# mumianyuxin/M3DSSD

Measured on AMD Instinct MI355X. Metric: images/sec at 1280x384 bs=8, 1/2/4/8 MI355X; 3D-box Linf vs ref, higher is better.
Workload: dtype f32; 1 GPU; BASELINE.json configs[1]: full M3d_inference_align (DLA-34 + DCNv2 align + ANAB) forward + decode + top-3000 + NMS, bs=8/GPU, 1280x384, fp32, random-init synthetic weights and frames; per_gpu_batch=8, global_batch=8, parallelism=dp1 (batch sharded, 1 all-gather of [B,40,14] detections)

## Files before the change

### include/m3dssd_hip.h

```cpp
#ifndef M3DSSD_HIP_H
#define M3DSSD_HIP_H

#include <stdint.h>

#ifdef __cplusplus
extern "C" {
#endif

typedef void *m3d_stream_t;

enum {
    M3D_OK = 0,
    M3D_E_ARG = -1,
    M3D_E_HIP = -2,
    M3D_E_WORKSPACE = -3
};

const char *m3d_last_error(void);
#define M3D_ABI_VERSION 5
int m3d_abi_version(void);
const char *m3d_source_hashes(void);

typedef struct m3d_conv_desc {
    const float *in;
// ... 9 lines not shown
    int out_nchw;
    long long out_img_stride;
    const float *scale;
    const float *shift;
    const float *res;
    int res_cs;
    int res_mode;
    int act;
    int sigmoid_from;
    const float *dcn_offmask;
    int dcn_om_cs;
    float *splitk_ws;
    long long splitk_ws_bytes;
} m3d_conv_desc;

int m3d_conv2d_forward(const m3d_conv_desc *d, m3d_stream_t stream);
int m3d_conv2d_splitk_plan(const m3d_conv_desc *d, int *splits, long long *ws_bytes);

int m3d_conv_wave_applicable(const m3d_conv_desc *d);
int m3d_conv_wave_splitk_plan(const m3d_conv_desc *d, int *splits, long long *ws_bytes);
int m3d_conv_wave_forward(const m3d_conv_desc *d, m3d_stream_t stream);
int m3d_conv_wave_forward_wgsplit(const m3d_conv_desc *d, m3d_stream_t stream);
int m3d_conv_wave_wgsplit_width(const m3d_conv_desc *d, int *slices, int *width);

int m3d_wino_conv3x3_forward(const m3d_conv_desc *d, m3d_stream_t stream);
int m3d_wino_conv3x3_variant(const m3d_conv_desc *d);
int m3d_wino_conv3x3_splitk_plan(const m3d_conv_desc *d, int *splits, long long *ws_bytes);
int m3d_wino_conv3x3_forward_ex(const m3d_conv_desc *d, int variant, m3d_stream_t stream);
int m3d_wino44_applicable(const m3d_conv_desc *d);
int m3d_wino44_conv3x3_forward(const m3d_conv_desc *d, m3d_stream_t stream);
int m3d_wino44_conv3x3_forward_ex(const m3d_conv_desc *d, int nb, m3d_stream_t stream);
int m3d_wino44_kpair(const m3d_conv_desc *d);
int m3d_wino44_splitk_plan(const m3d_conv_desc *d, int *splits, long long *ws_bytes);
int m3d_wino44_conv3x3_forward_touch(const m3d_conv_desc *d, int nb, const void *touch, long long touch_bytes, m3d_stream_t stream);

int m3d_cache_touch(const void *p, long long bytes, m3d_stream_t stream);
int m3d_upload_indirect(const void *const *src_slot, void *dst, long long bytes, m3d_stream_t stream);

int m3d_conv2d_tile(const m3d_conv_desc *d, int *bm, int *bn, int *bk, int *grid);

typedef struct m3d_conv_bf16_desc {
    const void *in;
    int in_cs;
    int N, H, W, Cin;
    const void *wgt;
    long long wgt_img_stride;
// ... 355 lines not shown
```

### m3dssd_amd/_hip.py

```python
import ctypes
import os
import subprocess

_HERE = os.path.dirname(os.path.abspath(__file__))
CSRC = os.path.join(_HERE, "csrc")
SO_PATH = os.environ.get("M3D_HIP_LIB") or os.path.join(CSRC, "build", "libm3dssd_hip.so")
HEADER = os.path.join(os.path.dirname(_HERE), "include", "m3dssd_hip.h")

c_int, c_float, c_ll, c_void_p = ctypes.c_int, ctypes.c_float, ctypes.c_longlong, ctypes.c_void_p


class ConvDesc(ctypes.Structure):
    _fields_ = [
        ("inp", c_void_p), ("in_cs", c_int),
        ("N", c_int), ("H", c_int), ("W", c_int), ("Cin", c_int),
        ("wgt", c_void_p), ("wgt_img_stride", c_ll),
        ("Cout", c_int), ("Cout_pad", c_int),
        ("kh", c_int), ("kw", c_int), ("stride", c_int), ("pad", c_int), ("dil", c_int),
        ("Ho", c_int), ("Wo", c_int),
        ("out", c_void_p), ("out_cs", c_int), ("out_nchw", c_int), ("out_img_stride", c_ll),
        ("scale", c_void_p), ("shift", c_void_p),
        ("res", c_void_p), ("res_cs", c_int), ("res_mode", c_int),
        ("act", c_int), ("sigmoid_from", c_int),
        ("dcn_offmask", c_void_p), ("dcn_om_cs", c_int),
# ... 109 lines not shown
    "m3d_upsample2x_add_bf16": (c_int, [P, c_int, P, P, c_int, P, c_int] + [c_int] * 4 + [P]),
    "m3d_f32_to_bf16": (c_int, [P, P, c_ll, P]),
    "m3d_softmax_rows_bf16": (c_int, [P, c_int, c_int, c_int, P, c_int, P]),
    "m3d_head_mlp_forward": (c_int, [ctypes.POINTER(MlpDesc), P]),
    "m3d_head_mlp_forward_batched": (c_int, [ctypes.POINTER(MlpDesc), c_int, P]),
    "m3d_head_mlp_forward_rows": (c_int, [ctypes.POINTER(MlpDesc), c_int, P, P, ctypes.c_uint, P]),
    "m3d_wino_conv3x3_forward": (c_int, [ctypes.POINTER(ConvDesc), P]),
    "m3d_wino_conv3x3_forward_ex": (c_int, [ctypes.POINTER(ConvDesc), c_int, P]),
    "m3d_wino_conv3x3_splitk_plan": (c_int, [ctypes.POINTER(ConvDesc), ctypes.POINTER(c_int), ctypes.POINTER(c_ll)]),
    "m3d_wino_conv3x3_variant": (c_int, [ctypes.POINTER(ConvDesc)]),
    "m3d_wino44_applicable": (c_int, [ctypes.POINTER(ConvDesc)]),
    "m3d_wino44_conv3x3_forward": (c_int, [ctypes.POINTER(ConvDesc), P]),
    "m3d_wino44_conv3x3_forward_ex": (c_int, [ctypes.POINTER(ConvDesc), c_int, P]),
    "m3d_wino44_kpair": (c_int, [ctypes.POINTER(ConvDesc)]),
    "m3d_wino44_conv3x3_forward_touch": (c_int, [ctypes.POINTER(ConvDesc), c_int, P, c_ll, P]),
    "m3d_cache_touch": (c_int, [P, c_ll, P]),
    "m3d_upload_indirect": (c_int, [P, P, c_ll, P]),
    "m3d_wino44_splitk_plan": (c_int, [ctypes.POINTER(ConvDesc), ctypes.POINTER(c_int), ctypes.POINTER(c_ll)]),
    "m3d_conv_wave_applicable": (c_int, [ctypes.POINTER(ConvDesc)]),
    "m3d_conv_wave_splitk_plan": (c_int, [ctypes.POINTER(ConvDesc), ctypes.POINTER(c_int), ctypes.POINTER(c_ll)]),
    "m3d_conv_wave_forward": (c_int, [ctypes.POINTER(ConvDesc), P]),
    "m3d_conv_wave_forward_wgsplit": (c_int, [ctypes.POINTER(ConvDesc), P]),
    "m3d_conv_wave_wgsplit_width": (c_int, [ctypes.POINTER(ConvDesc), ctypes.POINTER(c_int), ctypes.POINTER(c_int)]),
    "m3d_conv2d_tile": (c_int, [ctypes.POINTER(ConvDesc)] + [ctypes.POINTER(c_int)] * 4),
    "m3d_conv2d_splitk_plan": (c_int, [ctypes.POINTER(ConvDesc), ctypes.POINTER(c_int), ctypes.POINTER(c_ll)]),
    "m3d_dcn_v2_workspace_bytes": (c_ll, [c_int] * 10),
    "m3d_dcn_v2_workspace_bytes_grouped": (c_ll, [c_int] * 11),
    "m3d_dcn_v2_forward": (c_int, [P] * 6 + [c_int] * 14 + [P, c_ll, P]),
    "m3d_dcn_v2_backward_workspace_bytes": (c_ll, [c_int] * 11),
    "m3d_dcn_v2_backward": (c_int, [P] * 10 + [c_int] * 14 + [P, c_ll, P]),
    "m3d_dcn_v2_workspace_bytes_bf16": (c_ll, [c_int] * 11),
    "m3d_dcn_v2_forward_bf16": (c_int, [P, P, P, P, c_int, P, c_int, P] + [c_int] * 14 + [P, c_ll, P]),
    "m3d_dcn_v2_backward_workspace_bytes_bf16": (c_ll, [c_int] * 11),
    "m3d_dcn_v2_backward_bf16": (c_int, [P, P, P, c_int, P, c_int, P] + [P] * 5 + [c_int] * 14 + [P, c_ll, P]),
    "m3d_dcn_v2_psroi_pooling_workspace_bytes": (c_ll, [c_int] * 10),
    "m3d_dcn_v2_psroi_pooling_forward": (c_int, [P] * 5 + [c_int] * 8 + [c_float] + [c_int] * 5 + [c_float, P, c_ll, P]),
    "m3d_dcn_v2_psroi_pooling_backward": (c_int, [P] * 6 + [c_int] * 8 + [c_float] + [c_int] * 5 + [c_float, P, c_ll, P]),
    "m3d_rpn_loss_workspace_bytes": (c_ll, [c_int, c_ll]),
    "m3d_rpn_targets": (c_int, [P, c_int, c_int, c_int, P, c_int, P, c_int, c_int, P, P, c_int, P, P, P, P, P, c_ll, P]),
    "m3d_rpn_loss": (c_int, [P, c_int, c_int, c_int, P, c_int, P, c_int, c_int, P, P, P, c_int, P, P, P, P, P, P, P, P, P, P, c_ll, P]),
    "m3d_pack_conv_weight": (c_int, [P, P] + [c_int] * 6 + [P]),
    "m3d_nchw_to_nhwc": (c_int, [P, P] + [c_int] * 5 + [P]),
    "m3d_nhwc_to_nchw": (c_int, [P, c_int, P] + [c_int] * 4 + [P]),
    "m3d_stem_conv7x7": (c_int, [P, P, P, P, P] + [c_int] * 4 + [P]),
    "m3d_refine_3d": (c_int, [P, P, c_int, c_int, P, P, ctypes.c_double, c_int, ctypes.c_double, ctypes.c_double, P, P]),
    "m3d_refine_3d_ex": (c_int, [P, P, c_int, c_int, P, P, P, P, ctypes.c_double, c_int, ctypes.c_double, ctypes.c_double, P, P]),
# ... 96 lines not shown
```

### m3dssd_amd/csrc/dcn_wave.hip

```cpp

#include <type_traits>

#include "common.h"

struct ConvWaveArgs {
    const float *in, *wfrag, *scale, *shift, *res, *om;
    float *out;
    int in_cs, out_cs, res_cs, om_cs;
    int H, W, Cin, Ho, Wo, HoWo, Cout;
    int kh, kw, stride, pad, dil;
    int M, KG, tiles_n;
    int act, res_mode, sigmoid_from;
    int vec_out;
    long long w_img_stride;
    unsigned in_bytes, out_bytes, res_bytes, w_bytes;
    float *ws;
    int splits, ss_per, base_waves;
    unsigned ws_bytes;
#ifdef CONV_TRACE
    long long *trace;
#endif
};


#ifdef CONV_TRACE
static long long *g_conv_trace = nullptr;
extern "C" void m3d_conv_wave_set_trace(void *buf) { g_conv_trace = (long long *)buf; }
static int g_conv_variant = 0;
extern "C" void m3d_conv_wave_set_variant(int v) { g_conv_variant = v; }
#define TRACE_INIT() long long *trp = (a.trace && threadIdx.x < 64) ? a.trace + (size_t)blockIdx.x * 128 : nullptr; int tri = 0
#define TRACE() do { if (trp && lane == 0 && tri < 128) trp[tri++] = __builtin_readcyclecounter(); } while (0)
#else
#define TRACE_INIT()
#define TRACE()
#endif

template <bool DEFORM, int NT, int NCQ = 4, int WPE = (DEFORM ? 2 : 3), int S = 1>
__global__ __launch_bounds__(64 * S) __attribute__((amdgpu_waves_per_eu(WPE))) void conv_wave_kernel(const ConvWaveArgs a)
{
    __shared__ __attribute__((aligned(16))) float tileS[S * 32 * 32];
    __shared__ __attribute__((aligned(16))) float tapst[(DEFORM ? 9 : 1) * 32 * 8];
    const int lane = threadIdx.x & 63, l31 = lane & 31, h = lane >> 5;
    const int wv = S > 1 ? __builtin_amdgcn_readfirstlane((int)threadIdx.x >> 6) : 0;
    float *const tileA = tileS + wv * 1024;
    const int gp = lane >> 3, gc = lane & 7;
    TRACE_INIT();
    TRACE();
    int blk;
    {
        const int nblk = gridDim.x, bid = blockIdx.x;
        const int q = nblk >> 3, r = nblk & 7, xcd = bid & 7, loc = bid >> 3;
        blk = (xcd < r ? xcd * (q + 1) : r * (q + 1) + (xcd - r) * q) + loc;
    }
    int split = wv;
    if (S == 1 && a.splits > 1) {
        split = blk / a.base_waves;
        blk -= split * a.base_waves;
    }
    const int bm = blk / a.tiles_n, bn = blk - bm * a.tiles_n;
    const int m0 = bm * 32;
    const int KK = a.kh * a.kw, C32 = a.Cin / 32;
    const bool idle = S > 1 && wv >= a.splits;
// ... 255 lines not shown
                    const float *p = &tileS[px[q] * 32 + 4 * c4];
                    f32x4 v = *reinterpret_cast<const f32x4 *>(p);
#pragma unroll
                    for (int s = 1; s < S; ++s)
                        if (s < a.splits) v = v + *reinterpret_cast<const f32x4 *>(p + s * 1024);
                    v = conv_epi_affine(v, scv[nt], shv[nt], a.res ? rv[q] : v, a.res != nullptr, a.res_mode);
                    v = conv_epi_act4(v, c, a.sigmoid_from, tile_sig, slope);
                    if (full) {
                        __builtin_amdgcn_raw_buffer_store_b128(__builtin_bit_cast(u32x4, v), rout, oq[q] + (unsigned)c * 4u, 0, 0);
                    } else {
#pragma unroll
                        for (int e = 0; e < 4; ++e) {
                            const float pe = v[e];
                            __builtin_amdgcn_raw_buffer_store_b32(__builtin_bit_cast(unsigned, pe), rout,
                                                                  c + e < a.Cout ? oq[q] + (unsigned)(c + e) * 4u : M3D_BUF_OOB, 0, 0);
                        }
                    }
                }
            }
        }
        TRACE();
        return;
    }
    if (a.splits > 1) {
        const __amdgpu_buffer_rsrc_t rws = make_rsrc(a.ws, a.ws_bytes);
        const unsigned sbase = (unsigned)split * (unsigned)a.M;
        const unsigned cpad = (unsigned)(a.tiles_n * 32 * NT);
#pragma unroll
        for (int nt = 0; nt < NT; ++nt) {
            const unsigned co = (unsigned)(n0 + nt * 32 + l31);
#pragma unroll
            for (int r = 0; r < 16; ++r) {
                const int m = mb + (r & 3) + 8 * (r >> 2);
                const unsigned oo = m < a.M ? ((sbase + (unsigned)m) * cpad + co) * 4u : M3D_BUF_OOB;
                const float pv = acc[nt][r];
                __builtin_amdgcn_raw_buffer_store_b32(__builtin_bit_cast(unsigned, pv), rws, oo, 0, 0);
            }
        }
        return;
    }
    if (a.vec_out) {
        const float slope = a.act == 1 ? M3D_LEAKY_SLOPE : 1.f;
        const int pr = lane >> 3, c4 = lane & 7;
        unsigned oq[4], rq[4];
#pragma unroll
        for (int q = 0; q < 4; ++q) {
            const int m = m0 + pr + 8 * q;
            oq[q] = m < a.M ? (unsigned)m * (unsigned)a.out_cs * 4u : M3D_BUF_OOB;
            rq[q] = m < a.M ? (unsigned)m * (unsigned)a.res_cs * 4u : M3D_BUF_OOB;
        }
        f32x4 scv[NT], shv[NT];
#pragma unroll
        for (int nt = 0; nt < NT; ++nt) {
            const int c = n0 + nt * 32 + 4 * c4;
            scv[nt] = f32x4{1.f, 1.f, 1.f, 1.f};
            shv[nt] = f32x4{0.f, 0.f, 0.f, 0.f};
            if (c + 3 < a.Cout) {
                if (a.scale) scv[nt] = *reinterpret_cast<const f32x4 *>(a.scale + c);
                if (a.shift) shv[nt] = *reinterpret_cast<const f32x4 *>(a.shift + c);
            } else {
#pragma unroll
                for (int e = 0; e < 4; ++e)
                    if (c + e < a.Cout) {
                        if (a.scale) scv[nt][e] = a.scale[c + e];
                        if (a.shift) shv[nt][e] = a.shift[c + e];
                    }
            }
        }
#pragma unroll
        for (int nt = 0; nt < NT; ++nt) {
            const int c = n0 + nt * 32 + 4 * c4;
            f32x4 rv[4];
            if (a.res) {
#pragma unroll
                for (int q = 0; q < 4; ++q) {
                    if (c + 3 < a.Cout) {
                        rv[q] = __builtin_bit_cast(f32x4, __builtin_amdgcn_raw_buffer_load_b128(rres, rq[q] + (unsigned)c * 4u, 0, 0));
                    } else {
#pragma unroll
                        for (int e = 0; e < 4; ++e)
                            rv[q][e] = __builtin_bit_cast(float, __builtin_amdgcn_raw_buffer_load_b32(
                                rres, c + e < a.Cout ? rq[q] + (unsigned)(c + e) * 4u : M3D_BUF_OOB, 0, 0));
                    }
                }
            }
#pragma unroll
            for (int r = 0; r < 16; ++r) tileA[((r & 3) + 8 * (r >> 2) + 4 * h) * 32 + l31] = acc[nt][r];
            const bool tile_sig = a.sigmoid_from >= 0 && n0 + nt * 32 + 31 >= a.sigmoid_from;
#pragma unroll
            for (int q = 0; q < 4; ++q) {
                f32x4 v = *reinterpret_cast<const f32x4 *>(&tileA[(pr + 8 * q) * 32 + 4 * c4]);
                v = conv_epi_affine(v, scv[nt], shv[nt], a.res ? rv[q] : v, a.res != nullptr, a.res_mode);
                v = conv_epi_act4(v, c, a.sigmoid_from, tile_sig, slope);
                if (c + 3 < a.Cout) {
                    __builtin_amdgcn_raw_buffer_store_b128(__builtin_bit_cast(u32x4, v), rout, oq[q] + (unsigned)c * 4u, 0, 0);
                } else {
#pragma unroll
                    for (int e = 0; e < 4; ++e) {
                        const float pe = v[e];
                        __builtin_amdgcn_raw_buffer_store_b32(__builtin_bit_cast(unsigned, pe), rout,
                                                              c + e < a.Cout ? oq[q] + (unsigned)(c + e) * 4u : M3D_BUF_OOB, 0, 0);
                    }
                }
            }
        }
        TRACE();
        return;
    }
#pragma unroll
    for (int nt = 0; nt < NT; ++nt) {
        const int co = n0 + nt * 32 + l31;
        const bool cok = co < a.Cout;
        const float sc = (cok && a.scale) ? a.scale[co] : 1.f;
        const float sh = (cok && a.shift) ? a.shift[co] : 0.f;
        float rv[16];
        if (a.res) {
#pragma unroll
            for (int r = 0; r < 16; ++r) {
                const int m = mb + (r & 3) + 8 * (r >> 2);
                const unsigned ro = (cok && m < a.M) ? ((unsigned)m * (unsigned)a.res_cs + (unsigned)co) * 4u : M3D_BUF_OOB;
                rv[r] = __builtin_bit_cast(float, __builtin_amdgcn_raw_buffer_load_b32(rres, ro, 0, 0));
            }
        }
#pragma unroll
        for (int r = 0; r < 16; ++r) {
            const int m = mb + (r & 3) + 8 * (r >> 2);
            float v = conv_epi_affine(acc[nt][r], sc, sh, a.res ? rv[r] : 0.f, a.res != nullptr, a.res_mode);
            v = conv_epi_act(v, a.sigmoid_from >= 0 && co >= a.sigmoid_from, a.act == 1 ? M3D_LEAKY_SLOPE : 1.f);
            const unsigned oo = (cok && m < a.M) ? ((unsigned)m * (unsigned)a.out_cs + (unsigned)co) * 4u : M3D_BUF_OOB;
            __builtin_amdgcn_raw_buffer_store_b32(__builtin_bit_cast(unsigned, v), rout, oo, 0, 0);
        }
    }
    TRACE();
}

static int conv_wave_plan(const m3d_conv_desc *d, bool enforce_min, int *splits, int *ss_per, bool allow32 = false)
{
    *splits = 1;
    *ss_per = d->kh * d->kw * (d->Cin / 32);
    if (d->out_nchw) return 0;
    if (d->dcn_offmask && d->kh * d->kw > 9) return 0;
    if (d->Cin % 32 != 0 || d->Cout_pad % 32 != 0) return 0;
    if (d->Cout_pad % 64 != 0 && (!allow32 || d->dcn_offmask || d->wgt_img_stride)) return 0;
    const int cw = d->Cout_pad % 128 == 0 ? 128 : (d->Cout_pad % 64 == 0 ? 64 : 32);
    if (d->wgt_img_stride && (d->Ho * d->Wo) % 32 != 0) return 0;
    const long long M = (long long)d->N * d->Ho * d->Wo;
    const long long base = ((M + 31) / 32) * (d->Cout_pad / cw);
    if (base >= (1ll << 28)) return 0;
    static const int wave_min = m3d_env_int("M3D_CONV_WAVE_MIN", 900);
    static const int dcn_min = m3d_env_int("M3D_DCN_WAVE_MIN", 1500);
    static const int splitk = m3d_env_int("M3D_CONV_WAVE_SPLITK", 1);
    const long long need = d->dcn_offmask ? dcn_min : wave_min;
    const int nss = *ss_per;
    if (base < need && splitk && d->splitk_ws) {
        int s = (int)((1800 + base - 1) / base);
        if (s > nss / 4) s = nss / 4;
// ... 6 lines not shown
    if (enforce_min && base * *splits < need) { *splits = 1; *ss_per = nss; return 0; }
    return (int)(base * *splits);
}

extern "C" int m3d_conv_wave_applicable(const m3d_conv_desc *d)
{
    int s, p;
    return d ? conv_wave_plan(d, true, &s, &p) : 0;
}

extern "C" int m3d_conv_wave_splitk_plan(const m3d_conv_desc *d, int *splits, long long *ws_bytes)
{
    M3D_REQUIRE(d && splits && ws_bytes, "conv_wave_splitk_plan: null pointer");
    m3d_conv_desc t = *d;
    static float dummy;
    t.splitk_ws = &dummy;
    int p;
    const int waves = conv_wave_plan(&t, true, splits, &p, true);
    if (waves == 0) *splits = 1;
    *ws_bytes = (*splits > 1 && d->Cout_pad % 64 == 0) ? (long long)*splits * d->N * d->Ho * d->Wo * d->Cout_pad * 4 : 0;
    return M3D_OK;
}

template <bool DEFORM, int NT>
static void launch_wgsplit(const ConvWaveArgs &a, int S, int wgs, hipStream_t stream)
{
    constexpr int WPE = DEFORM ? 2 : 3;
    switch (S) {
    case 2: hipLaunchKernelGGL((conv_wave_kernel<DEFORM, NT, 4, WPE, 2>), dim3(wgs), dim3(128), 0, stream, a); break;
    case 4: hipLaunchKernelGGL((conv_wave_kernel<DEFORM, NT, 4, WPE, 4>), dim3(wgs), dim3(256), 0, stream, a); break;
    default: hipLaunchKernelGGL((conv_wave_kernel<DEFORM, NT, 4, WPE, 8>), dim3(wgs), dim3(512), 0, stream, a); break;
    }
}

static int conv_wave_run(const m3d_conv_desc *d_, hipStream_t stream, bool wgsplit)
{
    M3D_REQUIRE(d_ && d_->in && d_->wgt && d_->out, "conv_wave: null pointer");
    m3d_conv_desc dd = *d_;
    static float dummy;
    if (wgsplit) { dd.splitk_ws = &dummy; dd.splitk_ws_bytes = 0; }
    const m3d_conv_desc *d = &dd;
    int splits = 1, ss_per = 0;
    const int waves = conv_wave_plan(d, false, &splits, &ss_per, wgsplit);
    M3D_REQUIRE(waves > 0, "conv_wave: needs Cin %% 32 == 0, Cout_pad %% 64 == 0 (%% 32: plain, shared weights, wgsplit entry), NHWC output, "
                           "Ho*Wo %% 32 == 0 with per-image weights");
    const int ho = (d->H + 2 * d->pad - (d->dil * (d->kh - 1) + 1)) / d->stride + 1;
    const int wo = (d->W + 2 * d->pad - (d->dil * (d->kw - 1) + 1)) / d->stride + 1;
    M3D_REQUIRE(ho == d->Ho && wo == d->Wo, "conv_wave: Ho/Wo mismatch");
    M3D_REQUIRE(d->in_cs % 32 == 0 && d->in_cs >= d->Cin && ((uintptr_t)d->in & 127) == 0 && ((uintptr_t)d->wgt & 15) == 0,
                "conv_wave: the input view must be 128-byte aligned with in_cs %% 32 == 0");
    const long long M = (long long)d->N * d->Ho * d->Wo;
    M3D_REQUIRE(!d->wgt_img_stride || (d->wgt_img_stride % 4 == 0 && d->stride == 1 && d->Ho == d->H && d->Wo == d->W),
                "conv_wave: per-image weights need an image-aligned 16-byte stride and a same-size output");
    M3D_REQUIRE((long long)d->N * d->H * d->W * d->in_cs * 4 < (1ll << 31) && M * d->out_cs * 4 < (1ll << 31) &&
                M * d->res_cs * 4 < (1ll << 31) && (long long)d->Cout_pad * d->kh * d->kw * d->Cin * 4 < (1ll << 31),
                "conv_wave: views must be < 2 GiB");
    ConvWaveArgs a;
    a.in = d->in; a.wfrag = d->wgt; a.scale = d->scale; a.shift = d->shift; a.res = d->res; a.om = d->dcn_offmask;
    a.out = d->out;
    a.in_cs = d->in_cs; a.out_cs = d->out_cs; a.res_cs = d->res_cs; a.om_cs = d->dcn_om_cs;
    a.H = d->H; a.W = d->W; a.Cin = d->Cin; a.Ho = d->Ho; a.Wo = d->Wo; a.HoWo = d->Ho * d->Wo; a.Cout = d->Cout;
    a.kh = d->kh; a.kw = d->kw; a.stride = d->stride; a.pad = d->pad; a.dil = d->dil;
    const int cw = d->Cout_pad % 128 == 0 ? 128 : (d->Cout_pad % 64 == 0 ? 64 : 32);
    a.M = (int)M; a.KG = d->kh * d->kw * d->Cin / 8; a.tiles_n = d->Cout_pad / cw;
    a.act = d->act; a.res_mode = d->res_mode; a.sigmoid_from = d->sigmoid_from; a.w_img_stride = d->wgt_img_stride;
    static const int vec_epi = m3d_env_int("M3D_WAVE_VEC_EPILOGUE", 1);
    a.vec_out = vec_epi && d->out_cs % 4 == 0 && ((uintptr_t)d->out & 15) == 0 &&
                (!d->res || (d->res_cs % 4 == 0 && ((uintptr_t)d->res & 15) == 0)) &&
                (!d->scale || ((uintptr_t)d->scale & 15) == 0) && (!d->shift || ((uintptr_t)d->shift & 15) == 0);
    a.in_bytes = (unsigned)((long long)d->N * d->H * d->W * d->in_cs * 4);
    a.out_bytes = (unsigned)(M * d->out_cs * 4);
    a.res_bytes = (unsigned)(M * d->res_cs * 4);
    a.w_bytes = (unsigned)((long long)cw * d->kh * d->kw * d->Cin * 4);
#ifdef CONV_TRACE
    a.trace = g_conv_trace;
#endif
    a.ws = nullptr; a.splits = 1; a.ss_per = ss_per; a.base_waves = waves; a.ws_bytes = 0;
    if (splits > 1 && wgsplit) {
        const int S = splits <= 2 ? 2 : (splits <= 4 ? 4 : 8);
        M3D_REQUIRE(splits <= 8, "conv_wave: %d K slices do not fit a workgroup", splits);
        a.splits = splits; a.base_waves = waves / splits;
        if (cw == 128) {
            if (d->dcn_offmask) launch_wgsplit<true, 4>(a, S, a.base_waves, stream);
            else launch_wgsplit<false, 4>(a, S, a.base_waves, stream);
        } else if (cw == 64) {
            if (d->dcn_offmask) launch_wgsplit<true, 2>(a, S, a.base_waves, stream);
            else launch_wgsplit<false, 2>(a, S, a.base_waves, stream);
        } else {
            launch_wgsplit<false, 1>(a, S, a.base_waves, stream);
        }
        M3D_LAUNCH_CHECK();
        return M3D_OK;
    }
    if (splits > 1) {
        const long long need = (long long)splits * M * d->Cout_pad * 4;
        M3D_REQUIRE(need <= d->splitk_ws_bytes && need < (1ll << 31) && ((uintptr_t)d->splitk_ws & 15) == 0,
                    "conv_wave: split-K workspace too small (%lld bytes, see m3d_conv_wave_splitk_plan), >= 2 GiB or misaligned",
                    d->splitk_ws_bytes);
        a.ws = d->splitk_ws; a.splits = splits; a.base_waves = waves / splits; a.ws_bytes = (unsigned)need;
    }
// ... 32 lines not shown

extern "C" int m3d_conv_wave_forward(const m3d_conv_desc *d, m3d_stream_t stream)
{
    return conv_wave_run(d, (hipStream_t)stream, false);
}

extern "C" int m3d_conv_wave_wgsplit_width(const m3d_conv_desc *d, int *slices, int *width)
{
    M3D_REQUIRE(d && slices && width, "conv_wave_wgsplit_width: null pointer");
    m3d_conv_desc t = *d;
    static float dummy;
    t.splitk_ws = &dummy;
    int p;
    const int waves = conv_wave_plan(&t, false, slices, &p, true);
    M3D_REQUIRE(waves > 0 && *slices <= 8, "conv_wave_wgsplit_width: the wave kernel does not apply to this descriptor");
    *width = *slices <= 1 ? 1 : (*slices <= 2 ? 2 : (*slices <= 4 ? 4 : 8));
    return M3D_OK;
}

extern "C" int m3d_conv_wave_forward_wgsplit(const m3d_conv_desc *d, m3d_stream_t stream)
{
    return conv_wave_run(d, (hipStream_t)stream, true);
}
```

### m3dssd_amd/engine.py

```python
import ctypes
import math
import os

import numpy as np
import torch

from . import _hip
from ._hip import ConvDesc, MlpDesc
from .config import model_flags

BN_EPS = 1e-5
SELECT_KEYS = os.environ.get("M3D_SELECT_KEYS", "1") != "0"
SPARSE_HEADS_MAX_FRACTION = 0.5
PSP_SIZES = (1, 4, 8, 16)
BACKBONE_CHANNELS = {"dla34": (16, 32, 64, 128, 256, 512), "dla102": (16, 32, 128, 256, 512, 1024)}
DLA102_LEVELS = (1, 1, 1, 3, 4, 1)


def _rup(a, b):
    return (a + b - 1) // b * b


class View:
    __slots__ = ("t", "ptr", "n", "h", "w", "c", "cs", "keep")
# ... 482 lines not shown
        l0 = self._buf(plan, B, H, W, 16, name="level0")
        if P.get("level0.wino44") is not None and H % 4 == 0 and W % 4 == 0 and os.environ.get("M3D_LEVEL0_WINO44", "1") != "0":
            pc0 = P["level0"]
            self._op(plan, "level0", "wino44_c16", lambda st: _hip.check(L.m3d_conv3x3_c16_wino(
                s0.ptr, s0.cs, P["level0.wino44"].data_ptr(), pc0.scale.data_ptr(), pc0.shift.data_ptr(), l0.ptr, l0.cs,
                B, H, W, st)), flops=2.0 * B * H * W * 16 * 144, nbytes=B * H * W * 32 * 4)
        elif P["level0.direct"] is not None and os.environ.get("M3D_LEVEL0_IGEMM", "0") != "1":
            pc0 = P["level0"]
            self._op(plan, "level0", "conv3x3_c16", lambda st: _hip.check(L.m3d_conv3x3_c16(
                s0.ptr, s0.cs, P["level0.direct"].data_ptr(), pc0.scale.data_ptr(), pc0.shift.data_ptr(), l0.ptr, l0.cs,
                B, H, W, st)), flops=2.0 * B * H * W * 16 * 144, nbytes=B * H * W * 32 * 4)
        else:
            self._conv(plan, "level0", P["level0"], s0, l0, 1, 1, act=1)
        l1 = self._buf(plan, B, H // 2, W // 2, 32, name="level1")
        self._conv(plan, "level1", P["level1"], l0, l1, 2, 1, act=1)

        def maxpool(name, x, out):
            self._op(plan, name, "maxpool", lambda st: _hip.check(L.m3d_maxpool2x2(
                x.ptr, x.cs, out.ptr, out.cs, x.n, x.h, x.w, x.c, st)), nbytes=x.n * x.h * x.w * x.c * 5)

        if self.back_bone == "dla102":
            l3, l4, l5 = self._dla102_levels(plan, l1, maxpool)
        else:
            def block(p, x, res, out, stride):
                co = P[p + ".conv1"].cout
                t = self._buf(plan, B, out.h, out.w, co)
                self._conv(plan, p + ".conv1", P[p + ".conv1"], x, t, stride, 1, act=1)
                self._conv(plan, p + ".conv2", P[p + ".conv2"], t, out, 1, 1, act=1, res=res)

            def tree1(p, x, co, stride, out, bottom=None):
                h, w = x.h // stride, x.w // stride
                cat = self._buf(plan, B, h, w, 2 * co)
                x2v, x1v = cat.slice(0, co), cat.slice(co, co)
                if stride == 1:
                    bottom = x
                elif bottom is None:
                    bottom = self._buf(plan, B, h, w, x.c)
                    maxpool(p + ".downsample", x, bottom)
                if (p + ".project") in P:
                    res = self._buf(plan, B, h, w, co)
                    self._conv(plan, p + ".project", P[p + ".project"], bottom, res, 1, 0, act=0)
                else:
                    res = bottom
                block(p + ".tree1", x, res, x1v, stride)
                block(p + ".tree2", x1v, x1v, x2v, 1)
                self._conv(plan, p + ".root", P[p + ".root"], cat, out, 1, 0, act=1)

            l2 = self._buf(plan, B, H // 4, W // 4, 64, name="level2")
            tree1(b + ".level2", l1, 64, 2, l2)

            def tree2(p, x, co, out):
                ci = x.c
                h, w = x.h // 2, x.w // 2
                catb = self._buf(plan, B, h, w, 2 * co + ci + co)
                bottom = catb.slice(2 * co, ci)
                X1 = catb.slice(2 * co + ci, co)
                maxpool(p + ".downsample", x, bottom)
                tree1(p + ".tree1", x, co, 2, X1, bottom=bottom)
                x2v, x1v = catb.slice(0, co), catb.slice(co, co)
                block(p + ".tree2.tree1", X1, X1, x1v, 1)
                block(p + ".tree2.tree2", x1v, x1v, x2v, 1)
                self._conv(plan, p + ".tree2.root", P[p + ".tree2.root"], catb, out, 1, 0, act=1)

            l3 = self._buf(plan, B, H // 8, W // 8, 128, name="level3")
            tree2(b + ".level3", l2, 128, l3)
            l4 = self._buf(plan, B, H // 16, W // 16, 256, name="level4")
            tree2(b + ".level4", l3, 256, l4)
            l5 = self._buf(plan, B, H // 32, W // 32, 512, name="level5")
            h5, w5 = H // 32, W // 32
            cat5 = self._buf(plan, B, h5, w5, 1024 + 256)
            bottom5 = cat5.slice(1024, 256)
            maxpool(b + ".level5.downsample", l4, bottom5)
            res5 = self._buf(plan, B, h5, w5, 512)
            self._conv(plan, b + ".level5.project", P[b + ".level5.project"], bottom5, res5, 1, 0, act=0)
            block(b + ".level5.tree1", l4, res5, cat5.slice(512, 512), 2)
            block(b + ".level5.tree2", cat5.slice(512, 512), cat5.slice(512, 512), cat5.slice(0, 512), 1)
            self._conv(plan, b + ".level5.root", P[b + ".level5.root"], cat5, l5, 1, 0, act=1)

        def deform(p, x, out):
            om = self._buf(plan, B, x.h, x.w, 27, 28)
            self._conv(plan, p + ".offset_mask", P[p + ".om"], x, om, 1, 1, act=0, sigmoid_from=18)
# ... 493 lines not shown
```

Measured before the change: 1556 images/sec.

## Fuse DLA tree entry maxpool, 1x1 projection and stride-2 conv1 into one kernel

Adds an ENTRY variant of the wave conv kernel that runs the stride-2 3x3 conv1 and then, in a second pass, builds the 2x2 max-pooled input from the conv1 gather taps. It feeds that pooled tile straight into the 1x1 projection MFMA and optionally writes the pooled map when a later concat needs it. This replaces three launches (maxpool, project, conv1) with one and avoids writing and re-reading the pooled map when it is only used internally. The cost is a longer and more complex kernel with higher register pressure, and it only applies to unsplit plans with even H and W; otherwise the three-launch path is kept.

```diff
diff --git a/include/m3dssd_hip.h b/include/m3dssd_hip.h
--- a/include/m3dssd_hip.h
+++ b/include/m3dssd_hip.h
@@ -55,6 +55,8 @@
 int m3d_conv_wave_forward(const m3d_conv_desc *d, m3d_stream_t stream);
 int m3d_conv_wave_forward_wgsplit(const m3d_conv_desc *d, m3d_stream_t stream);
 int m3d_conv_wave_wgsplit_width(const m3d_conv_desc *d, int *slices, int *width);
+int m3d_conv_wave_tree_entry_forward(const m3d_conv_desc *conv1, const m3d_conv_desc *project, float *bottom, int bottom_cs,
+                                     m3d_stream_t stream);
 
 int m3d_wino_conv3x3_forward(const m3d_conv_desc *d, m3d_stream_t stream);
 int m3d_wino_conv3x3_variant(const m3d_conv_desc *d);
diff --git a/m3dssd_amd/_hip.py b/m3dssd_amd/_hip.py
--- a/m3dssd_amd/_hip.py
+++ b/m3dssd_amd/_hip.py
@@ -155,6 +155,7 @@
     "m3d_conv_wave_forward": (c_int, [ctypes.POINTER(ConvDesc), P]),
     "m3d_conv_wave_forward_wgsplit": (c_int, [ctypes.POINTER(ConvDesc), P]),
     "m3d_conv_wave_wgsplit_width": (c_int, [ctypes.POINTER(ConvDesc), ctypes.POINTER(c_int), ctypes.POINTER(c_int)]),
+    "m3d_conv_wave_tree_entry_forward": (c_int, [ctypes.POINTER(ConvDesc), ctypes.POINTER(ConvDesc), P, c_int, P]),
     "m3d_conv2d_tile": (c_int, [ctypes.POINTER(ConvDesc)] + [ctypes.POINTER(c_int)] * 4),
     "m3d_conv2d_splitk_plan": (c_int, [ctypes.POINTER(ConvDesc), ctypes.POINTER(c_int), ctypes.POINTER(c_ll)]),
     "m3d_dcn_v2_workspace_bytes": (c_ll, [c_int] * 10),
diff --git a/m3dssd_amd/csrc/dcn_wave.hip b/m3dssd_amd/csrc/dcn_wave.hip
--- a/m3dssd_amd/csrc/dcn_wave.hip
+++ b/m3dssd_amd/csrc/dcn_wave.hip
@@ -22,6 +22,18 @@
 #endif
 };
 
+struct ConvEntryArgs : ConvWaveArgs {
+    const float *p_wfrag, *p_scale, *p_shift;
+    float *p_out, *bottom;
+    int p_out_cs, bottom_cs, p_KG, p_vec_out;
+    unsigned p_out_bytes, bottom_bytes, p_w_bytes;
+};
+
+struct ConvWaveEpi {
+    const float *scale, *shift, *res;
+    int out_cs, res_cs, act, res_mode, sigmoid_from, vec_out;
+};
+
 
 #ifdef CONV_TRACE
 static long long *g_conv_trace = nullptr;
@@ -35,9 +47,12 @@
 #define TRACE()
 #endif
 
-template <bool DEFORM, int NT, int NCQ = 4, int WPE = (DEFORM ? 2 : 3), int S = 1>
-__global__ __launch_bounds__(64 * S) __attribute__((amdgpu_waves_per_eu(WPE))) void conv_wave_kernel(const ConvWaveArgs a)
-{
+template <bool DEFORM, int NT, int NCQ = 4, int WPE = (DEFORM ? 2 : 3), int S = 1, bool ENTRY = false>
+__global__ __launch_bounds__(64 * S) __attribute__((amdgpu_waves_per_eu(WPE))) void conv_wave_kernel(
+    const std::conditional_t<ENTRY, ConvEntryArgs, ConvWaveArgs> ka)
+{
+    static_assert(!ENTRY || (!DEFORM && S == 1), "the tree entry is a plain, unsplit kernel");
+    const ConvWaveArgs &a = ka;
     __shared__ __attribute__((aligned(16))) float tileS[S * 32 * 32];
     __shared__ __attribute__((aligned(16))) float tapst[(DEFORM ? 9 : 1) * 32 * 8];
     const int lane = threadIdx.x & 63, l31 = lane & 31, h = lane >> 5;
@@ -339,7 +354,7 @@
         TRACE();
         return;
     }
-    if (a.splits > 1) {
+    if (!ENTRY && a.splits > 1) {
         const __amdgpu_buffer_rsrc_t rws = make_rsrc(a.ws, a.ws_bytes);
         const unsigned sbase = (unsigned)split * (unsigned)a.M;
         const unsigned cpad = (unsigned)(a.tiles_n * 32 * NT);
@@ -356,99 +371,197 @@
         }
         return;
     }
-    if (a.vec_out) {
-        const float slope = a.act == 1 ? M3D_LEAKY_SLOPE : 1.f;
-        const int pr = lane >> 3, c4 = lane & 7;
-        unsigned oq[4], rq[4];
-#pragma unroll
-        for (int q = 0; q < 4; ++q) {
-            const int m = m0 + pr + 8 * q;
-            oq[q] = m < a.M ? (unsigned)m * (unsigned)a.out_cs * 4u : M3D_BUF_OOB;
-            rq[q] = m < a.M ? (unsigned)m * (unsigned)a.res_cs * 4u : M3D_BUF_OOB;
-        }
-        f32x4 scv[NT], shv[NT];
+    ConvWaveEpi ep{a.scale, a.shift, a.res, a.out_cs, a.res_cs, a.act, a.res_mode, a.sigmoid_from, a.vec_out};
+    __amdgpu_buffer_rsrc_t eout = rout, eres = rres;
+#pragma unroll
+    for (int pass = 0; pass < (ENTRY ? 2 : 1); ++pass) {
+        if constexpr (ENTRY) {
+            if (pass == 1) {
+                typedef const ConvEntryArgs __attribute__((address_space(4))) *EntryArgsPtr;
+                EntryArgsPtr kp = (EntryArgsPtr)__builtin_amdgcn_kernarg_segment_ptr();
+                asm volatile("" : "+s"(kp));
+                const __amdgpu_buffer_rsrc_t rwp = make_rsrc(kp->p_wfrag + (size_t)bn * NT * kp->p_KG * 256, kp->p_w_bytes);
+                const unsigned pwstride = (unsigned)kp->p_KG * 1024u;
+                const bool wr_bottom = kp->bottom != nullptr && bn == 0;
+                const __amdgpu_buffer_rsrc_t rbot = make_rsrc(wr_bottom ? kp->bottom : a.out, wr_bottom ? kp->bottom_bytes : 0u);
+                int m0e = m0, le = lane;
+                asm volatile("" : "+s"(m0e), "+v"(le));
+                const int gpe = le >> 3, gce = le & 7, l31e = le & 31, he = le >> 5;
+                unsigned bq[4];
+#pragma unroll
+                for (int g = 0; g < 4; ++g) {
+                    const int m = m0e + 8 * g + gpe;
+                    g_valid[g] = m < kp->M;
+                    const int mm = g_valid[g] ? m : 0;
+                    const int n = mm / kp->HoWo, rem = mm - n * kp->HoWo;
+                    const int ho = rem / kp->Wo, wo = rem - ho * kp->Wo;
+                    g_pix[g] = n * kp->H * kp->W;
+                    g_hi0[g] = ho * 2 - 1;
+                    g_wi0[g] = wo * 2 - 1;
+                    bq[g] = g_valid[g] ? ((unsigned)m * (unsigned)kp->bottom_cs + (unsigned)gce * 4u) * 4u : M3D_BUF_OOB;
+                    const int r = 8 * g + gpe;
+                    wr_off[g] = (unsigned)(r * 32 + ((gce ^ ((r >> 1) & 7)) * 4));
+                }
+#pragma unroll
+                for (int j = 0; j < 4; ++j) rd_off[j] = (unsigned)(l31e * 32 + (((2 * j + he) ^ ((l31e >> 1) & 7)) * 4));
+                auto issue_pb = [&](int kg, f32x4 (&bf)[NT]) {
+                    const unsigned bsoff = (unsigned)min(kg, kp->p_KG - 1) * 1024u;
+#pragma unroll
+                    for (int nt = 0; nt < NT; ++nt) bf[nt] = buf_load_f32x4(rwp, wlane, bsoff + nt * pwstride);
+                };
+#pragma unroll
+                for (int nt = 0; nt < NT; ++nt)
+#pragma unroll
+                    for (int r = 0; r < 16; ++r) acc[nt][r] = 0.f;
+                for (int c = 0; c < C32; ++c) {
+                    f32x4 top[4], bot[4];
+                    setup_tap(4);
+                    issue_gather(c);
+#pragma unroll
+                    for (int g = 0; g < 4; ++g) top[g] = cr[g][0];
+                    setup_tap(5);
+                    issue_gather(c);
+#pragma unroll
+                    for (int g = 0; g < 4; ++g)
+#pragma unroll
+                        for (int e = 0; e < 4; ++e) top[g][e] = fmaxf(top[g][e], cr[g][0][e]);
+                    setup_tap(7);
+                    issue_gather(c);
+#pragma unroll
+                    for (int g = 0; g < 4; ++g) bot[g] = cr[g][0];
+                    setup_tap(8);
+                    issue_gather(c);
+#pragma unroll
+                    for (int g = 0; g < 4; ++g) {
+                        f32x4 v;
+#pragma unroll
+                        for (int e = 0; e < 4; ++e) v[e] = fmaxf(top[g][e], fmaxf(bot[g][e], cr[g][0][e]));
+                        if (wr_bottom) buf_store_f32x4_nop(v, rbot, bq[g], (unsigned)c * 128u);
+                        *reinterpret_cast<f32x4 *>(&tileA[wr_off[g]]) = v;
+                    }
+                    f32x4 A[4];
+#pragma unroll
+                    for (int j = 0; j < 4; ++j) A[j] = *reinterpret_cast<const f32x4 *>(&tileA[rd_off[j]]);
+                    issue_pb(c * 4, bfA);
+                    __builtin_amdgcn_sched_barrier(0);
+                    auto pgroup = [&](int j, f32x4 (&bf)[NT], f32x4 (&bfn)[NT]) {
+                        if (j < 3) issue_pb(c * 4 + j + 1, bfn);
+                        __builtin_amdgcn_sched_barrier(0);
+#pragma unroll
+                        for (int t = 0; t < 4; ++t)
+#pragma unroll
+                            for (int nt = 0; nt < NT; ++nt)
+                                acc[nt] = __builtin_amdgcn_mfma_f32_32x32x2f32(A[j][t], bf[nt][t], acc[nt], 0, 0, 0);
+                        __builtin_amdgcn_sched_barrier(0);
+                    };
+                    pgroup(0, bfA, bfB);
+                    pgroup(1, bfB, bfA);
+                    pgroup(2, bfA, bfB);
+                    pgroup(3, bfB, bfA);
+                }
+                ep = ConvWaveEpi{kp->p_scale, kp->p_shift, nullptr, kp->p_out_cs, 0, 0, 0, -1, kp->p_vec_out};
+                eout = make_rsrc(kp->p_out, kp->p_out_bytes);
+                eres = make_rsrc(kp->p_out, 0u);
+            }
+        }
+        int el = lane, em0 = m0, en0 = n0;
+        if constexpr (ENTRY) asm volatile("" : "+v"(el), "+s"(em0), "+s"(en0));
+        const int el31 = el & 31, eh = el >> 5, emb = em0 + 4 * eh;
+        if (ep.vec_out) {
+            const float slope = ep.act == 1 ? M3D_LEAKY_SLOPE : 1.f;
+            const int pr = el >> 3, c4 = el & 7;
+            unsigned oq[4], rq[4];
+#pragma unroll
+            for (int q = 0; q < 4; ++q) {
+                const int m = em0 + pr + 8 * q;
+                oq[q] = m < a.M ? (unsigned)m * (unsigned)ep.out_cs * 4u : M3D_BUF_OOB;
+                rq[q] = m < a.M ? (unsigned)m * (unsigned)ep.res_cs * 4u : M3D_BUF_OOB;
+            }
+            f32x4 scv[NT], shv[NT];
+#pragma unroll
+            for (int nt = 0; nt < NT; ++nt) {
+                const int c = en0 + nt * 32 + 4 * c4;
+                scv[nt] = f32x4{1.f, 1.f, 1.f, 1.f};
+                shv[nt] = f32x4{0.f, 0.f, 0.f, 0.f};
+                if (c + 3 < a.Cout) {
+                    if (ep.scale) scv[nt] = *reinterpret_cast<const f32x4 *>(ep.scale + c);
+                    if (ep.shift) shv[nt] = *reinterpret_cast<const f32x4 *>(ep.shift + c);
+                } else {
+#pragma unroll
+                    for (int e = 0; e < 4; ++e)
+                        if (c + e < a.Cout) {
+                            if (ep.scale) scv[nt][e] = ep.scale[c + e];
+                            if (ep.shift) shv[nt][e] = ep.shift[c + e];
+                        }
+                }
+            }
+#pragma unroll
+            for (int nt = 0; nt < NT; ++nt) {
+                const int c = en0 + nt * 32 + 4 * c4;
+                f32x4 rv[4];
+                if (ep.res) {
+#pragma unroll
+                    for (int q = 0; q < 4; ++q) {
+                        if (c + 3 < a.Cout) {
+                            rv[q] = __builtin_bit_cast(f32x4, __builtin_amdgcn_raw_buffer_load_b128(eres, rq[q] + (unsigned)c * 4u, 0, 0));
+                        } else {
+#pragma unroll
+                            for (int e = 0; e < 4; ++e)
+                                rv[q][e] = __builtin_bit_cast(float, __builtin_amdgcn_raw_buffer_load_b32(
+                                    eres, c + e < a.Cout ? rq[q] + (unsigned)(c + e) * 4u : M3D_BUF_OOB, 0, 0));
+                        }
+                    }
+                }
+#pragma unroll
+                for (int r = 0; r < 16; ++r) tileA[((r & 3) + 8 * (r >> 2) + 4 * eh) * 32 + el31] = acc[nt][r];
+                const bool tile_sig = ep.sigmoid_from >= 0 && en0 + nt * 32 + 31 >= ep.sigmoid_from;
+#pragma unroll
+                for (int q = 0; q < 4; ++q) {
+                    f32x4 v = *reinterpret_cast<const f32x4 *>(&tileA[(pr + 8 * q) * 32 + 4 * c4]);
+                    v = conv_epi_affine(v, scv[nt], shv[nt], ep.res ? rv[q] : v, ep.res != nullptr, ep.res_mode);
+                    v = conv_epi_act4(v, c, ep.sigmoid_from, tile_sig, slope);
+                    if (c + 3 < a.Cout) {
+                        __builtin_amdgcn_raw_buffer_store_b128(__builtin_bit_cast(u32x4, v), eout, oq[q] + (unsigned)c * 4u, 0, 0);
+                    } else {
+#pragma unroll
+                        for (int e = 0; e < 4; ++e) {
+                            const float pe = v[e];
+                            __builtin_amdgcn_raw_buffer_store_b32(__builtin_bit_cast(unsigned, pe), eout,
+                                                                  c + e < a.Cout ? oq[q] + (unsigned)(c + e) * 4u : M3D_BUF_OOB, 0, 0);
+                        }
+                    }
+                }
+            }
+            TRACE();
+            if constexpr (!ENTRY) return;
+            else continue;
+        }
 #pragma unroll
         for (int nt = 0; nt < NT; ++nt) {
-            const int c = n0 + nt * 32 + 4 * c4;
-            scv[nt] = f32x4{1.f, 1.f, 1.f, 1.f};
-            shv[nt] = f32x4{0.f, 0.f, 0.f, 0.f};
-            if (c + 3 < a.Cout) {
-                if (a.scale) scv[nt] = *reinterpret_cast<const f32x4 *>(a.scale + c);
-                if (a.shift) shv[nt] = *reinterpret_cast<const f32x4 *>(a.shift + c);
-            } else {
-#pragma unroll
-                for (int e = 0; e < 4; ++e)
-                    if (c + e < a.Cout) {
-                        if (a.scale) scv[nt][e] = a.scale[c + e];
-                        if (a.shift) shv[nt][e] = a.shift[c + e];
-                    }
-            }
-        }
-#pragma unroll
-        for (int nt = 0; nt < NT; ++nt) {
-            const int c = n0 + nt * 32 + 4 * c4;
-            f32x4 rv[4];
-            if (a.res) {
-#pragma unroll
-                for (int q = 0; q < 4; ++q) {
-                    if (c + 3 < a.Cout) {
-                        rv[q] = __builtin_bit_cast(f32x4, __builtin_amdgcn_raw_buffer_load_b128(rres, rq[q] + (unsigned)c * 4u, 0, 0));
-                    } else {
-#pragma unroll
-                        for (int e = 0; e < 4; ++e)
-                            rv[q][e] = __builtin_bit_cast(float, __builtin_amdgcn_raw_buffer_load_b32(
-                                rres, c + e < a.Cout ? rq[q] + (unsigned)(c + e) * 4u : M3D_BUF_OOB, 0, 0));
-                    }
-                }
-            }
-#pragma unroll
-            for (int r = 0; r < 16; ++r) tileA[((r & 3) + 8 * (r >> 2) + 4 * h) * 32 + l31] = acc[nt][r];
-            const bool tile_sig = a.sigmoid_from >= 0 && n0 + nt * 32 + 31 >= a.sigmoid_from;
-#pragma unroll
-            for (int q = 0; q < 4; ++q) {
-                f32x4 v = *reinterpret_cast<const f32x4 *>(&tileA[(pr + 8 * q) * 32 + 4 * c4]);
-                v = conv_epi_affine(v, scv[nt], shv[nt], a.res ? rv[q] : v, a.res != nullptr, a.res_mode);
-                v = conv_epi_act4(v, c, a.sigmoid_from, tile_sig, slope);
-                if (c + 3 < a.Cout) {
-                    __builtin_amdgcn_raw_buffer_store_b128(__builtin_bit_cast(u32x4, v), rout, oq[q] + (unsigned)c * 4u, 0, 0);
-                } else {
-#pragma unroll
-                    for (int e = 0; e < 4; ++e) {
-                        const float pe = v[e];
-                        __builtin_amdgcn_raw_buffer_store_b32(__builtin_bit_cast(unsigned, pe), rout,
-                                                              c + e < a.Cout ? oq[q] + (unsigned)(c + e) * 4u : M3D_BUF_OOB, 0, 0);
-                    }
-                }
+            const int co = en0 + nt * 32 + el31;
+            const bool cok = co < a.Cout;
+            const float sc = (cok && ep.scale) ? ep.scale[co] : 1.f;
+            const float sh = (cok && ep.shift) ? ep.shift[co] : 0.f;
+            float rv[16];
+            if (ep.res) {
+#pragma unroll
+                for (int r = 0; r < 16; ++r) {
+                    const int m = emb + (r & 3) + 8 * (r >> 2);
+                    const unsigned ro = (cok && m < a.M) ? ((unsigned)m * (unsigned)ep.res_cs + (unsigned)co) * 4u : M3D_BUF_OOB;
+                    rv[r] = __builtin_bit_cast(float, __builtin_amdgcn_raw_buffer_load_b32(eres, ro, 0, 0));
+                }
+            }
+#pragma unroll
+            for (int r = 0; r < 16; ++r) {
+                const int m = emb + (r & 3) + 8 * (r >> 2);
+                float v = conv_epi_affine(acc[nt][r], sc, sh, ep.res ? rv[r] : 0.f, ep.res != nullptr, ep.res_mode);
+                v = conv_epi_act(v, ep.sigmoid_from >= 0 && co >= ep.sigmoid_from, ep.act == 1 ? M3D_LEAKY_SLOPE : 1.f);
+                const unsigned oo = (cok && m < a.M) ? ((unsigned)m * (unsigned)ep.out_cs + (unsigned)co) * 4u : M3D_BUF_OOB;
+                __builtin_amdgcn_raw_buffer_store_b32(__builtin_bit_cast(unsigned, v), eout, oo, 0, 0);
             }
         }
         TRACE();
-        return;
-    }
-#pragma unroll
-    for (int nt = 0; nt < NT; ++nt) {
-        const int co = n0 + nt * 32 + l31;
-        const bool cok = co < a.Cout;
-        const float sc = (cok && a.scale) ? a.scale[co] : 1.f;
-        const float sh = (cok && a.shift) ? a.shift[co] : 0.f;
-        float rv[16];
-        if (a.res) {
-#pragma unroll
-            for (int r = 0; r < 16; ++r) {
-                const int m = mb + (r & 3) + 8 * (r >> 2);
-                const unsigned ro = (cok && m < a.M) ? ((unsigned)m * (unsigned)a.res_cs + (unsigned)co) * 4u : M3D_BUF_OOB;
-                rv[r] = __builtin_bit_cast(float, __builtin_amdgcn_raw_buffer_load_b32(rres, ro, 0, 0));
-            }
-        }
-#pragma unroll
-        for (int r = 0; r < 16; ++r) {
-            const int m = mb + (r & 3) + 8 * (r >> 2);
-            float v = conv_epi_affine(acc[nt][r], sc, sh, a.res ? rv[r] : 0.f, a.res != nullptr, a.res_mode);
-            v = conv_epi_act(v, a.sigmoid_from >= 0 && co >= a.sigmoid_from, a.act == 1 ? M3D_LEAKY_SLOPE : 1.f);
-            const unsigned oo = (cok && m < a.M) ? ((unsigned)m * (unsigned)a.out_cs + (unsigned)co) * 4u : M3D_BUF_OOB;
-            __builtin_amdgcn_raw_buffer_store_b32(__builtin_bit_cast(unsigned, v), rout, oo, 0, 0);
-        }
-    }
-    TRACE();
+    }
 }
 
 static int conv_wave_plan(const m3d_conv_desc *d, bool enforce_min, int *splits, int *ss_per, bool allow32 = false)
@@ -501,28 +614,8 @@
     return M3D_OK;
 }
 
-template <bool DEFORM, int NT>
-static void launch_wgsplit(const ConvWaveArgs &a, int S, int wgs, hipStream_t stream)
-{
-    constexpr int WPE = DEFORM ? 2 : 3;
-    switch (S) {
-    case 2: hipLaunchKernelGGL((conv_wave_kernel<DEFORM, NT, 4, WPE, 2>), dim3(wgs), dim3(128), 0, stream, a); break;
-    case 4: hipLaunchKernelGGL((conv_wave_kernel<DEFORM, NT, 4, WPE, 4>), dim3(wgs), dim3(256), 0, stream, a); break;
-    default: hipLaunchKernelGGL((conv_wave_kernel<DEFORM, NT, 4, WPE, 8>), dim3(wgs), dim3(512), 0, stream, a); break;
-    }
-}
-
-static int conv_wave_run(const m3d_conv_desc *d_, hipStream_t stream, bool wgsplit)
-{
-    M3D_REQUIRE(d_ && d_->in && d_->wgt && d_->out, "conv_wave: null pointer");
-    m3d_conv_desc dd = *d_;
-    static float dummy;
-    if (wgsplit) { dd.splitk_ws = &dummy; dd.splitk_ws_bytes = 0; }
-    const m3d_conv_desc *d = &dd;
-    int splits = 1, ss_per = 0;
-    const int waves = conv_wave_plan(d, false, &splits, &ss_per, wgsplit);
-    M3D_REQUIRE(waves > 0, "conv_wave: needs Cin %% 32 == 0, Cout_pad %% 64 == 0 (%% 32: plain, shared weights, wgsplit entry), NHWC output, "
-                           "Ho*Wo %% 32 == 0 with per-image weights");
+static int conv_wave_args(const m3d_conv_desc *d, int ss_per, int waves, ConvWaveArgs &a)
+{
     const int ho = (d->H + 2 * d->pad - (d->dil * (d->kh - 1) + 1)) / d->stride + 1;
     const int wo = (d->W + 2 * d->pad - (d->dil * (d->kw - 1) + 1)) / d->stride + 1;
     M3D_REQUIRE(ho == d->Ho && wo == d->Wo, "conv_wave: Ho/Wo mismatch");
@@ -534,7 +627,6 @@
     M3D_REQUIRE((long long)d->N * d->H * d->W * d->in_cs * 4 < (1ll << 31) && M * d->out_cs * 4 < (1ll << 31) &&
                 M * d->res_cs * 4 < (1ll << 31) && (long long)d->Cout_pad * d->kh * d->kw * d->Cin * 4 < (1ll << 31),
                 "conv_wave: views must be < 2 GiB");
-    ConvWaveArgs a;
     a.in = d->in; a.wfrag = d->wgt; a.scale = d->scale; a.shift = d->shift; a.res = d->res; a.om = d->dcn_offmask;
     a.out = d->out;
     a.in_cs = d->in_cs; a.out_cs = d->out_cs; a.res_cs = d->res_cs; a.om_cs = d->dcn_om_cs;
@@ -555,6 +647,35 @@
     a.trace = g_conv_trace;
 #endif
     a.ws = nullptr; a.splits = 1; a.ss_per = ss_per; a.base_waves = waves; a.ws_bytes = 0;
+    return M3D_OK;
+}
+
+template <bool DEFORM, int NT>
+static void launch_wgsplit(const ConvWaveArgs &a, int S, int wgs, hipStream_t stream)
+{
+    constexpr int WPE = DEFORM ? 2 : 3;
+    switch (S) {
+    case 2: hipLaunchKernelGGL((conv_wave_kernel<DEFORM, NT, 4, WPE, 2>), dim3(wgs), dim3(128), 0, stream, a); break;
+    case 4: hipLaunchKernelGGL((conv_wave_kernel<DEFORM, NT, 4, WPE, 4>), dim3(wgs), dim3(256), 0, stream, a); break;
+    default: hipLaunchKernelGGL((conv_wave_kernel<DEFORM, NT, 4, WPE, 8>), dim3(wgs), dim3(512), 0, stream, a); break;
+    }
+}
+
+static int conv_wave_run(const m3d_conv_desc *d_, hipStream_t stream, bool wgsplit)
+{
+    M3D_REQUIRE(d_ && d_->in && d_->wgt && d_->out, "conv_wave: null pointer");
+    m3d_conv_desc dd = *d_;
+    static float dummy;
+    if (wgsplit) { dd.splitk_ws = &dummy; dd.splitk_ws_bytes = 0; }
+    const m3d_conv_desc *d = &dd;
+    int splits = 1, ss_per = 0;
+    const int waves = conv_wave_plan(d, false, &splits, &ss_per, wgsplit);
+    M3D_REQUIRE(waves > 0, "conv_wave: needs Cin %% 32 == 0, Cout_pad %% 64 == 0 (%% 32: plain, shared weights, wgsplit entry), NHWC output, "
+                           "Ho*Wo %% 32 == 0 with per-image weights");
+    ConvWaveArgs a;
+    if (const int rc = conv_wave_args(d, ss_per, waves, a)) return rc;
+    const int cw = d->Cout_pad % 128 == 0 ? 128 : (d->Cout_pad % 64 == 0 ? 64 : 32);
+    const long long M = (long long)d->N * d->Ho * d->Wo;
     if (splits > 1 && wgsplit) {
         const int S = splits <= 2 ? 2 : (splits <= 4 ? 4 : 8);
         M3D_REQUIRE(splits <= 8, "conv_wave: %d K slices do not fit a workgroup", splits);
@@ -633,3 +754,47 @@
 {
     return conv_wave_run(d, (hipStream_t)stream, true);
 }
+
+extern "C" int m3d_conv_wave_tree_entry_forward(const m3d_conv_desc *c1, const m3d_conv_desc *pj, float *bottom, int bottom_cs,
+                                                m3d_stream_t stream)
+{
+    M3D_REQUIRE(c1 && pj && c1->in && c1->wgt && c1->out && pj->wgt && pj->out, "conv_wave_tree_entry: null pointer");
+    M3D_REQUIRE(c1->kh == 3 && c1->kw == 3 && c1->stride == 2 && c1->pad == 1 && c1->dil == 1 && !c1->dcn_offmask &&
+                !c1->wgt_img_stride && !c1->out_nchw,
+                "conv_wave_tree_entry: conv1 must be a plain 3x3 stride-2 pad-1 convolution with an NHWC output");
+    M3D_REQUIRE(pj->kh == 1 && pj->kw == 1 && pj->stride == 1 && pj->pad == 0 && pj->dil == 1 && !pj->dcn_offmask &&
+                !pj->wgt_img_stride && !pj->out_nchw && !pj->res && pj->act == 0 && pj->sigmoid_from < 0,
+                "conv_wave_tree_entry: the projection must be a plain 1x1 convolution without residual or activation");
+    M3D_REQUIRE(c1->H % 2 == 0 && c1->W % 2 == 0 && c1->H > 0 && c1->W > 0,
+                "conv_wave_tree_entry: H and W (%d x %d) must be even: the pool grid and the conv1 grid must coincide", c1->H, c1->W);
+    M3D_REQUIRE(pj->N == c1->N && pj->Cin == c1->Cin && pj->H == c1->Ho && pj->W == c1->Wo && pj->Ho == c1->Ho && pj->Wo == c1->Wo &&
+                pj->Cout == c1->Cout && pj->Cout_pad == c1->Cout_pad && c1->Ho == c1->H / 2 && c1->Wo == c1->W / 2,
+                "conv_wave_tree_entry: the descriptors disagree on input, N, Ho, Wo or Cout");
+    M3D_REQUIRE(!pj->in || (bottom && pj->in == bottom && pj->in_cs == bottom_cs),
+                "conv_wave_tree_entry: the projection's input must be the pooled map `bottom` (or NULL)");
+    int splits = 1, ss_per = 0, psplits = 1, pss = 0;
+    const int waves = conv_wave_plan(c1, false, &splits, &ss_per), pwaves = conv_wave_plan(pj, false, &psplits, &pss);
+    M3D_REQUIRE(waves > 0 && pwaves > 0 && waves / splits == pwaves / psplits,
+                "conv_wave_tree_entry: needs Cin %% 32 == 0, Cout_pad %% 64 == 0");
+    M3D_REQUIRE(splits == 1 && psplits == 1, "conv_wave_tree_entry: the plan splits K (conv1 %d, projection %d slices): run the three launches",
+                splits, psplits);
+    ConvEntryArgs a;
+    if (const int rc = conv_wave_args(c1, ss_per, waves, a)) return rc;
+    const long long M = (long long)c1->N * c1->Ho * c1->Wo;
+    const int cw = c1->Cout_pad % 128 == 0 ? 128 : 64;
+    M3D_REQUIRE(((uintptr_t)pj->wgt & 15) == 0 && M * pj->out_cs * 4 < (1ll << 31) && pj->out_cs >= pj->Cout,
+                "conv_wave_tree_entry: projection views must be < 2 GiB, the weights 16-byte aligned");
+    M3D_REQUIRE(!bottom || (bottom_cs % 4 == 0 && bottom_cs >= c1->Cin && ((uintptr_t)bottom & 15) == 0 && M * bottom_cs * 4 < (1ll << 31)),
+                "conv_wave_tree_entry: `bottom` must be 16-byte aligned with bottom_cs %% 4 == 0, < 2 GiB");
+    a.p_wfrag = pj->wgt; a.p_scale = pj->scale; a.p_shift = pj->shift; a.p_out = pj->out; a.bottom = bottom;
+    a.p_out_cs = pj->out_cs; a.bottom_cs = bottom ? bottom_cs : 0; a.p_KG = pj->Cin / 8;
+    a.p_vec_out = a.vec_out && pj->out_cs % 4 == 0 && ((uintptr_t)pj->out & 15) == 0 &&
+                  (!pj->scale || ((uintptr_t)pj->scale & 15) == 0) && (!pj->shift || ((uintptr_t)pj->shift & 15) == 0);
+    a.p_out_bytes = (unsigned)(M * pj->out_cs * 4);
+    a.bottom_bytes = bottom ? (unsigned)(M * bottom_cs * 4) : 0u;
+    a.p_w_bytes = (unsigned)((long long)cw * pj->Cin * 4);
+    if (cw == 128) hipLaunchKernelGGL((conv_wave_kernel<false, 4, 4, 3, 1, true>), dim3(waves), dim3(64), 0, (hipStream_t)stream, a);
+    else hipLaunchKernelGGL((conv_wave_kernel<false, 2, 4, 3, 1, true>), dim3(waves), dim3(64), 0, (hipStream_t)stream, a);
+    M3D_LAUNCH_CHECK();
+    return M3D_OK;
+}
diff --git a/m3dssd_amd/engine.py b/m3dssd_amd/engine.py
--- a/m3dssd_amd/engine.py
+++ b/m3dssd_amd/engine.py
@@ -528,27 +528,60 @@
         if self.back_bone == "dla102":
             l3, l4, l5 = self._dla102_levels(plan, l1, maxpool)
         else:
+            tree_entry_on = os.environ.get("M3D_TREE_ENTRY", "1") != "0"
+
             def block(p, x, res, out, stride):
                 co = P[p + ".conv1"].cout
                 t = self._buf(plan, B, out.h, out.w, co)
                 self._conv(plan, p + ".conv1", P[p + ".conv1"], x, t, stride, 1, act=1)
                 self._conv(plan, p + ".conv2", P[p + ".conv2"], t, out, 1, 1, act=1, res=res)
 
-            def tree1(p, x, co, stride, out, bottom=None):
+            def tree_entry(p, pool_name, x, bottom, own_bottom, res, t):
+                n0 = len(plan.ops)
+                self._conv(plan, p + ".project", P[p + ".project"], bottom, res, 1, 0, act=0)
+                self._conv(plan, p + ".tree1.conv1", P[p + ".tree1.conv1"], x, t, 2, 1, act=1)
+                new = plan.ops[n0:]
+                if (tree_entry_on and len(new) == 2 and all(op[1] == "conv_wave" for op in new)
+                        and x.h % 2 == 0 and x.w % 2 == 0 and x.c % 32 == 0):
+                    (_, _, fl_p, _, dp), (_, _, fl_c, _, dc) = new
+                    del plan.ops[n0:]
+                    bptr, bcs = (None, 0) if own_bottom else (bottom.ptr, bottom.cs)
+                    if own_bottom:
+                        dp.inp = None
+                        plan.keep[:] = [k for k in plan.keep if k is not bottom.t]
+                    rc, rp = ctypes.byref(dc), ctypes.byref(dp)
+                    m = x.n * t.h * t.w
+                    nbytes = 4 * (x.n * x.h * x.w * x.c + m * (2 * dc.Cout + (0 if own_bottom else x.c)) + dc.Cout * 10 * x.c)
+                    self._op(plan, p + ".entry", "conv_wave<entry>", lambda st: _hip.check(L.m3d_conv_wave_tree_entry_forward(
+                        rc, rp, bptr, bcs, st)), flops=fl_c + fl_p, nbytes=nbytes)
+                else:
+                    maxpool(pool_name, x, bottom)
+                    plan.ops.insert(n0, plan.ops.pop())
+
+            def tree1(p, x, co, stride, out, bottom=None, pool_name=None):
                 h, w = x.h // stride, x.w // stride
                 cat = self._buf(plan, B, h, w, 2 * co)
                 x2v, x1v = cat.slice(0, co), cat.slice(co, co)
+                own_bottom = False
                 if stride == 1:
                     bottom = x
                 elif bottom is None:
                     bottom = self._buf(plan, B, h, w, x.c)
-                    maxpool(p + ".downsample", x, bottom)
+                    own_bottom, pool_name = True, p + ".downsample"
                 if (p + ".project") in P:
                     res = self._buf(plan, B, h, w, co)
-                    self._conv(plan, p + ".project", P[p + ".project"], bottom, res, 1, 0, act=0)
+                    if stride == 2:
+                        t = self._buf(plan, B, h, w, co)
+                        tree_entry(p, pool_name, x, bottom, own_bottom, res, t)
+                        self._conv(plan, p + ".tree1.conv2", P[p + ".tree1.conv2"], t, x1v, 1, 1, act=1, res=res)
+                    else:
+                        self._conv(plan, p + ".project", P[p + ".project"], bottom, res, 1, 0, act=0)
+                        block(p + ".tree1", x, res, x1v, stride)
                 else:
+                    if pool_name is not None:
+                        maxpool(pool_name, x, bottom)
                     res = bottom
-                block(p + ".tree1", x, res, x1v, stride)
+                    block(p + ".tree1", x, res, x1v, stride)
                 block(p + ".tree2", x1v, x1v, x2v, 1)
                 self._conv(plan, p + ".root", P[p + ".root"], cat, out, 1, 0, act=1)
 
@@ -561,8 +594,7 @@
                 catb = self._buf(plan, B, h, w, 2 * co + ci + co)
                 bottom = catb.slice(2 * co, ci)
                 X1 = catb.slice(2 * co + ci, co)
-                maxpool(p + ".downsample", x, bottom)
-                tree1(p + ".tree1", x, co, 2, X1, bottom=bottom)
+                tree1(p + ".tree1", x, co, 2, X1, bottom=bottom, pool_name=p + ".downsample")
                 x2v, x1v = catb.slice(0, co), catb.slice(co, co)
                 block(p + ".tree2.tree1", X1, X1, x1v, 1)
                 block(p + ".tree2.tree2", x1v, x1v, x2v, 1)
```

After: 1555 images/sec. Within noise of the previous version (-0.1%).
